# goroda/c3sc

Measured on AMD Instinct MI355X. Metric: Bellman-sweep nodes/sec (7D car rank-10), higher is better.
Workload: dtype f64

## Files before the change

c3sc_amd/csrc/c3sc_hip.hip:

```cpp
#include <hip/hip_runtime.h>

#include <algorithm>
#include <cmath>
#include <cstdio>
#include <cstdlib>
#include <cstring>
#include <string>
#include <vector>

#include "../../include/c3sc_hip.h"
#include "fiber_partition.hpp"
#include "fiber_partition_sort.hpp"
#include "kernel_chain_walk.hpp"
#include "kernel_common.hpp"
#include "kernel_rollout.hpp"
#include "kernel_rollout_ode.hpp"
#include "model_tables.hpp"
#include "pad_cores.hpp"
#include "registry.hpp"

namespace c3sc {

std::vector<KernelEntry> &kernel_registry()
{
// ... 929 lines not shown
    A.h2 = c->h2;
    A.discount = c->discount;
    for (int i = 0; i < 2 * c->d; i++) A.t[i] = c->t[i];
    for (int i = 0; i < C3SC_MAX_PARAMS; i++) A.prm[i] = c->prm[i];
    A.status = c->d_status;
    A.game_gsz = c->game_gsz;
    A.game_ngrp = c->game_ngrp;
    A.game_order = c->game_order;
    A.hz_off = c->hz_dt > 0.0 ? c->hz_off : 0;
    {
        static const int dbg_env = [] { const char *e = getenv("C3SC_DBG"); return e ? atoi(e) : 0; }();
        A.dbg = dbg_env;
        if (dbg_env && !c->d_dbg) { HIPCHK(c, hipMalloc((void **)&c->d_dbg, 65536 * 8 * sizeof(unsigned long long))); }
        A.dbgbuf = c->d_dbg;
        if (A.dbg & 8) A.ncand = 1;
        if (A.dbg & 16) A.ncand = 3;
    }
    return C3SC_OK;
}

static void arm_memo(c3sc_hip_ctx *c, const KernelEntry *e, KArgs &A)
{
    A.memo_keys = nullptr;
    if (c->memo.keys == nullptr || e->variant != C3SC_VARIANT_FIBER_PER_WAVE) return;
    A.memo_keys = c->memo.keys; A.memo_vals = c->memo.vals; A.memo_capmask = c->memo.capmask; A.memo_epoch_bits = c->memo.epoch_bits;
    A.memo_shift = c->memo.shift; A.memo_counters = c->memo.counters; A.memo_mode = c->memo.mode;
    for (int m = 0; m < c->d; m++) A.memo_stride[m] = c->memo.stride[m];
    c->memo.applied = true;
}

static hipError_t ctx_launch(const c3sc_hip_ctx *c, const KernelEntry &e, const KArgs &A, LaunchIO io)
{
    io.form = c->switches;
    return launch_entry(e, A, io);
}

static int launch_one(c3sc_hip_ctx *c, const KernelEntry *e, const KArgs &A, const LaunchIO &io, const char *unsupported = nullptr)
{
    c->last_kernel = e->name;
    g_launches++;
    c->status_cache_valid = false;
    const hipError_t he = ctx_launch(c, *e, A, io);
    if (he == hipErrorNotSupported && unsupported) return fail(c, C3SC_ERR_UNSUPPORTED, unsupported);
    HIPCHK(c, he);
    return C3SC_OK;
}

constexpr long FIBER_PARTITION_MIN = 262144;
static long fiber_partition_min()
{
    const char *e = getenv("C3SC_FIBER_PARTITION");
    if (!e || !*e) return FIBER_PARTITION_MIN;
    const long v = atol(e);
    return v > 0 ? v : -1;
}

static long fiber_group_floor()
{
    const char *e = getenv("C3SC_FIBER_GROUP");
    if (!e || !*e) return FPART_MIN_PER_BIN;
    const long v = atol(e);
    return v > 0 ? v : -1;
}

static bool fiber_rank()
{
// ... 1041 lines not shown
```

c3sc_amd/csrc/inst_car7d_fpp.hip:

```cpp
#include "launch_fpw.hpp"
#include "launch_fpp.hpp"
#include "models.hpp"
namespace c3sc {
#define REG7P(RP)                                  \
    C3SC_REG_FPP1(C3SC_MODEL_CAR7D, RP, 0, Car7D)  \
    C3SC_REG_FPP1(C3SC_MODEL_CAR7D, RP, 1, Car7D)  \
    C3SC_REG_FPP1(C3SC_MODEL_CAR7D, RP, 2, Car7D)  \
    C3SC_REG_FPP1(C3SC_MODEL_CAR7D, RP, 3, Car7D)  \
    C3SC_REG_FPP1(C3SC_MODEL_CAR7D, RP, 4, Car7D)  \
    C3SC_REG_FPP1(C3SC_MODEL_CAR7D, RP, 5, Car7D)  \
    C3SC_REG_FPP1(C3SC_MODEL_CAR7D, RP, 6, Car7D)
#define CAR7_MAP(K, MERGED, NVEC)                                                                   \
    static_assert(PairPark<Car7D, K>::merged() == (MERGED), "car7d: merged dimensions of K = " #K); \
    static_assert(PairMap<Car7D, K>::nv() == (NVEC), "car7d: folded vectors of K = " #K);
CAR7_MAP(0, 0x1Eu, 5)
CAR7_MAP(1, 0x1Du, 6)
CAR7_MAP(2, 0x18u, 9)
CAR7_MAP(3, 0x04u, 11)
CAR7_MAP(4, 0x0Bu, 7)
CAR7_MAP(5, 0x0Fu, 5)
CAR7_MAP(6, 0x17u, 5)
C3SC_FPP_TABLE3(Car7D, 10)
#define CAR7_PLAN3(K, ROUNDS, PRODUCTS)                                                                                  \
    static_assert(PairMap<Car7D, K, true, true>::plan().staged == (ROUNDS), "car7d: three-core staging rounds of K = " #K); \
    static_assert(PairMap<Car7D, K, true, true>::plan().products == (PRODUCTS), "car7d: three-core products of K = " #K);
CAR7_PLAN3(0, 3, 24)
CAR7_PLAN3(1, 2, 16)
CAR7_PLAN3(2, 1, 8)
CAR7_PLAN3(3, 0, 0)
CAR7_PLAN3(4, 1, 6)
CAR7_PLAN3(5, 2, 8)
CAR7_PLAN3(6, 3, 16)
REG7P(4)
REG7P(10)
}
```

c3sc_amd/csrc/kernel_fiber_pair.hpp:

```cpp
#pragma once
#include <utility>

#include "fold_lds.hpp"

#ifndef FPP_CGD
#define FPP_CGD 3
#endif
#ifndef FPP_PIPE2
#define FPP_PIPE2 1
#endif
#ifndef FPP_CG
#define FPP_CG 1
#endif
#ifndef FPP_NV
#define FPP_NV 4
#endif

#ifndef FPP_DIRECT_MAXD
#define FPP_DIRECT_MAXD 3
#endif
#ifndef FPP_EDGE_TABLES
#define FPP_EDGE_TABLES 1
#endif

#ifndef FPP_NODE_SPLIT
#define FPP_NODE_SPLIT 1
#endif
#ifndef FPP_NODE_SPLIT_VGPRS
#define FPP_NODE_SPLIT_VGPRS 140
#endif

namespace c3sc {

constexpr int FPP_THREADS = 128;

template <class Model, int RP>
__host__ __device__ constexpr bool fpp_direct() { return Model::D <= FPP_DIRECT_MAXD && RP <= 8; }

template <class Model, int RP>
__host__ __device__ constexpr bool fpp_edge_tables() { return FPP_EDGE_TABLES && !fpp_direct<Model, RP>() && Model::D >= 4; }

template <int RP>
__device__ __forceinline__ void load_row16(const double *__restrict__ p, double (&r)[RP])
{
    typedef double v2d __attribute__((ext_vector_type(2)));
#pragma unroll
    for (int i = 0; i < RP / 2; i++) {
        const v2d v = *reinterpret_cast<const v2d *>(p + 2 * i);
        r[2 * i] = v.x;
        r[2 * i + 1] = v.y;
    }
}

template <int RP, int NW, int FIRST, int COUNT, bool ROWVEC>
__device__ inline void apply_core_and(const double *G, double (&W)[NW][RP], double (&E)[RP])
{
    constexpr int N1 = COUNT >= FPP_NV - 1 ? FPP_NV - 1 : COUNT;
    double tmp[N1 + 1][RP];
#pragma unroll
    for (int a = 0; a < RP; a++) tmp[0][a] = E[a];
#pragma unroll
    for (int s = 0; s < N1; s++)
// ... 249 lines not shown
    {
        if (PK::merged() == 0u) return pair_owner<K>(it);
        int load[2] = {0, 0}, own[NIT] = {};
        bool done[NIT] = {};
        for (int n = 0; n < NIT; n++) {
            int best = -1;
            for (int q = 0; q < NIT; q++)
                if (valid(q) && !done[q] && (best < 0 || cost(q) > cost(best))) best = q;
            if (best < 0) break;
            const int h = load[1] < load[0] ? 1 : 0;
            own[best] = h;
            load[h] += cost(best);
            done[best] = true;
        }
        return own[it];
    }
    template <int H>
    __host__ __device__ static constexpr int lslot(int it)
    {
        return (it == UL || it < K) ? SL::template slot<H>(it) : SR::template slot<H>(it);
    }
};

__host__ __device__ constexpr bool fpp_node_split_optout(int d, int rp, int k) { return rp < 10 || (d == 7 && rp == 10 && k == 4); }
template <class Model, int RP, int K>
__host__ __device__ constexpr bool fpp_node_split()
{
    if constexpr (!FPP_NODE_SPLIT || fpp_direct<Model, RP>()) return false;
    else
        return PairPark<Model, K>::merged() != 0u && PairMap<Model, K>::nv() * RP * 2 <= FPP_NODE_SPLIT_VGPRS &&
               !fpp_node_split_optout(Model::D, RP, K);
}

template <class Model, int K>
struct PairPre {
    static constexpr unsigned MASK = PairPark<Model, K>::merged(), RATES = PairPark<Model, K>::rates();
    const double *PX;
    int lane;
    double pvc;
    __device__ inline double q() const { return PX[PairPark<Model, K>::row_q() * 64 + lane]; }
    __device__ inline double pv() const { return pvc; }
    __device__ inline double pm(int m) const { return PX[PairPark<Model, K>::row_pm(m) * 64 + lane]; }
    __device__ inline double pp(int m) const { return PX[(PairPark<Model, K>::row_pm(m) + 1) * 64 + lane]; }
};

#define FPP_STAMP(slot)                                                   \
    if (C3SC_STAMPS_ON && (A.dbg & 128)) {                                \
        const unsigned long long now__ = clock64();                       \
        seg[slot] += now__ - tlast;                                       \
        tlast = now__;                                                    \
    }

template <class Model, int RP, int K, int H, bool PART, bool T3, bool LEFT, int m, int NOWN, class Combine>
__device__ __attribute__((always_inline)) inline void fold_step(const KArgs &A, const double *__restrict__ ro, double *sK,
                                                               const int (&fi)[Model::D], const int (&nbm)[Model::D], const int (&nbp)[Model::D],
                                                               const double (&rpm)[Model::D], const double (&rpp)[Model::D], double (&V)[RP],
                                                               double (&W)[NOWN][RP], unsigned long long (&seg)[12], unsigned long long &tlast,
                                                               Combine &&combine)
{
    constexpr int D = Model::D;
    constexpr bool DIRECT = fpp_direct<Model, RP>();
    typedef PairMap<Model, K, fpp_edge_tables<Model, RP>(), T3> PM;
    typedef typename PM::template Side<LEFT> SD;
    constexpr bool RV = SD::ROWVEC;
    constexpr int BASE = SD::template base<H>();
    constexpr KeyLevels KL = fpp_group_levels(D, RP, K);
// ... 29 lines not shown
                vecmat_lds<RP, 1>(src + nbm[m] * str, t0);
                vecmat_lds<RP, 1>(src + nbp[m] * str, t1);
            } else {
                matvec_lds<RP, 1>(src + nbm[m] * str, t0);
                matvec_lds<RP, 1>(src + nbp[m] * str, t1);
            }
#pragma unroll
            for (int a = 0; a < RP; a++) {
                if constexpr (PAIR) { W[BASE + before][a] = t0[0][a]; W[BASE + before + 1][a] = t1[0][a]; }
                else nw[a] = fma(rpp[m], t1[0][a], rpm[m] * t0[0][a]);
            }
        }
        if constexpr (DIRECT) {
            double tl[1][RP];
#pragma unroll
            for (int a = 0; a < RP; a++) tl[0][a] = V[a];
            apply_glb<RP, 1, RV>(G, tl);
#pragma unroll
            for (int a = 0; a < RP; a++) V[a] = tl[0][a];
            apply_range_glb<RP, NOWN, BASE, before, RV>(G, W);
        } else if constexpr (UNI)
            apply_uni_and<RP, NOWN, BASE, before, RV>(G, W, V);
        else
            apply_core_and<RP, NOWN, BASE, before, RV>(G, W, V);
        if constexpr (ACC) {
            constexpr int su = SD::template slot<H>(SD::U);
#pragma unroll
            for (int a = 0; a < RP; a++) W[su][a] = (m == SD::first_merged()) ? nw[a] : W[su][a] + nw[a];
        }
    };
    fold_level<GROUP && (m == KL.major || (KL.n > 1 && m == KL.minor))>(fi[m], body);
}

template <class Model, int RP, int K, int H, bool FORCED, bool PART, bool T3 = false>
__device__ __attribute__((always_inline)) inline void fiber_pair_body(const KArgs &A, const double *__restrict__ ro,
                                                                     const int32_t *__restrict__ idx, double *__restrict__ outv,
                                                                     int32_t *__restrict__ uidx, int32_t *__restrict__ absorbed,
                                                                     const int32_t *__restrict__ perm, const int32_t *__restrict__ nlive_p,
                                                                     double *sK, unsigned &st)
{
    constexpr int D = Model::D;
    constexpr int S = 2 * D + 1;
    constexpr int RH = RP / 2;
    typedef PairPark<Model, K> PK;
    constexpr bool ET = fpp_edge_tables<Model, RP>();
    typedef PairMap<Model, K, ET, T3> PM;
    static_assert(!T3 || (PART && ET), "the three-core tables serve the partitioned kernels with edge tables");
    static_assert(PM::nv() == PairMap<Model, K, ET>::nv() && PM::gslot(D + 1) == PairMap<Model, K, ET>::gslot(D + 1),
                  "the table depth moves no slot of the node loop");
    constexpr FoldPlan PL = PM::plan();
    constexpr int NV = PM::nv();
    constexpr int NVL = PM::SL::nv();
    constexpr int NOL = PM::SL::template before<H>(K);
    constexpr int NOR = PM::SR::template before<H>(K);
    constexpr int NOWN = (NOL + NOR) > 0 ? (NOL + NOR) : 1;
    constexpr int NP = NV + 1;
    constexpr bool DIRECT = fpp_direct<Model, RP>();
    constexpr KeyLevels KL = fpp_group_levels(D, RP, K);
    constexpr bool GROUP = PART && KL.n > 0;
    static_assert(!GROUP || fpp_key_levels(D, K, ET).major == KL.major, "the key levels follow the kernel's own fold plan");
    static_assert(RP % 2 == 0, "rank-split kernel needs an even padded rank");
    const int lane = threadIdx.x & 63;
    const int N = A.N;
    const long ntiles = (A.F + 63) / 64;
    int first_dead = 0x7fffffff;
    if constexpr (PART) first_dead = __builtin_amdgcn_readfirstlane((int)(((long)*nlive_p + 63) >> 6));
    unsigned long long seg[12] = {0, 0, 0, 0, 0, 0, 0, 0, 0, 0, 0, 0}, tlast = clock64();
    CandLds<Model> cr;
    NodeLds<Model, K> nr;
    {
        CandRegs<Model> cr0;
        cr0.load(A, ro);
        NodeRegs<Model, K> nr0;
        nr0.load(A, ro);
        double *tb = sK + A.tbl_off;
        cr.fill(tb, cr0, A.ncand);
        nr.fill(tb + CandLds<Model>::doubles(A.ncand), nr0, N);
        pair_barrier();
    }

    for (long tile = blockIdx.x; tile < ntiles; tile += gridDim.x) {
        FPP_STAMP(7)
        const long f_raw = tile * 64 + lane;
        const bool live = f_raw < A.F;
        const long f_pos = live ? f_raw : A.F - 1;
        long f = f_pos;
        if constexpr (PART) f = (long)perm[f_pos];
        const bool dead_tile = PART && tile >= (long)first_dead;

        if constexpr (PART) if (dead_tile) {
            const bool whole = A.bctype[K] == C3SC_ABSORB || A.cends != 0;
            const int jb = whole ? 0 : 1, je = whole ? N : N - 1;
            double xb[D];
#pragma unroll
            for (int m = 0; m < D; m++) xb[m] = (m != K && PK::need_x(m)) ? ro[A.xg_off[m] + idx[f * D + m]] : 0.0;
            for (int j = jb + ((jb ^ H) & 1); j < je; j += 2) {
                xb[K] = nr.x_at(j);
                outv[(size_t)f * N + j] = Model::boundcost(A.prm, xb);
                if (uidx) uidx[(size_t)f * N + j] = -1;
                if (absorbed) absorbed[(size_t)f * N + j] = 1;
            }
            if (whole) continue;
        }

        int fi[D], nbm[D], nbp[D];
        bool fiber_abs = false;
        double x[D];
#pragma unroll
        for (int m = 0; m < D; m++) {
            fi[m] = (m == K) ? 0 : idx[f * D + m];
            const bool face = fixed_neighbors(fi[m], A.ngrid[m], A.bctype[m], nbm[m], nbp[m]);
            if (m != K) fiber_abs = fiber_abs || face;
            x[m] = ro[A.xg_off[m] + fi[m]];
        }

        const unsigned obs_fixed = obstacle_mask_fixed<D>(A, ro, x, K);
        double tv[Model::NTAB > 0 ? Model::NTAB : 1];
        table_values<Model>(A, ro, fi, tv);

        double rpm[D], rpp[D];
#pragma unroll
        for (int m = 0; m < D; m++) { rpm[m] = 0.0; rpp[m] = 0.0; }
        if constexpr (PK::constd() != 0) {
            typename Model::Node nd0;
            Model::prep(A.prm, x, tv, nd0);
            double u0[Model::DU], cf0[Model::NCF > 0 ? Model::NCF : 1], b0[D], s0[D];
#pragma unroll
            for (int i = 0; i < Model::DU; i++) u0[i] = cr.get_u(i, 0);
            cf0[0] = 0.0;
#pragma unroll
            for (int i = 0; i < Model::NCF; i++) cf0[i] = cr.get_cf(i, 0);
            Model::drift(A.prm, nd0, x, u0, cf0, b0);
            Model::sigma(A.prm, x, u0, s0);
#pragma unroll
            for (int m = 0; m < D; m++)
                if ((PK::constd() >> m) & 1u) upwind_rates(A.t[2 * m], A.t[2 * m + 1], b0[m], s0[m], rpm[m], rpp[m]);
        }

        double L[RP], R[RP], W[NOWN][RP];
#pragma unroll
        for (int a = 0; a < RP; a++) { L[a] = (a == 0) ? 1.0 : 0.0; R[a] = (a == 0) ? 1.0 : 0.0; }

        auto side3 = [&](auto lc, double (&V)[RP]) __attribute__((always_inline)) {
            constexpr bool LEFT = decltype(lc)::value;
            typedef typename PM::template Side<LEFT> SD;
            constexpr int c0 = SD::core(0), c1 = SD::core(1), c2 = SD::core(2);
            constexpr int BASE = SD::template base<H>();
            const double *T = ro + (LEFT ? pair_tab3L_off(A, RP) : pair_tab3R_off(A, RP));
            const int n0 = A.ngrid[c0], n1 = A.ngrid[c1];
            auto row = [&](int j0, int j1, int j2) __attribute__((always_inline)) -> const double * {
                return T + (LEFT ? ((long)j2 * n0 + j0) * n1 + j1 : ((long)j2 * n1 + j1) * n0 + j0) * RP;
            };
            constexpr bool OWN0 = SD::template owns<H>(c0), OWN1 = SD::template owns<H>(c1), OWN2 = SD::template owns<H>(c2);
            double tm[3][RP], tp[3][RP];
            load_row16<RP>(row(fi[c0], fi[c1], fi[c2]), V);
            if constexpr (OWN0) {
                load_row16<RP>(row(nbm[c0], fi[c1], fi[c2]), tm[0]);
                load_row16<RP>(row(nbp[c0], fi[c1], fi[c2]), tp[0]);
            }
            if constexpr (OWN1) {
                load_row16<RP>(row(fi[c0], nbm[c1], fi[c2]), tm[1]);
                load_row16<RP>(row(fi[c0], nbp[c1], fi[c2]), tp[1]);
            }
            if constexpr (OWN2) {
                load_row16<RP>(row(fi[c0], fi[c1], nbm[c2]), tm[2]);
                load_row16<RP>(row(fi[c0], fi[c1], nbp[c2]), tp[2]);
            }
            __builtin_amdgcn_sched_barrier(0);
            auto combine = [&]() __attribute__((always_inline)) {
// ... 131 lines not shown
            if constexpr (PM::SR::tab() && K == PL.rfirst) right_combine();
            if constexpr (!PM::SR::tab()) {
                constexpr bool GLB = DIRECT || !PL.redge;
                constexpr int str = GLB ? RP : fpl_lds_stride(RP);
                const double *src = sK;
                FPP_STAMP(1)
                if constexpr (GLB) src = ro + A.core_off[D - 1];
                else {
                    pair_barrier();
                    stage_core_image<H>(sK, A.img_base + A.pair_img_off[D - 1], A.ngrid[D - 1] * str);
                    pair_barrier();
                }
                FPP_STAMP(7)
#pragma unroll
                for (int a = 0; a < RP; a++) {
                    R[a] = src[fi[D - 1] * str + a];
                    if constexpr (PM::mg(D - 1)) {
                        if constexpr (PM::owner(PM::UR) == H)
                            W[NOL][a] = fma(rpp[D - 1], src[nbp[D - 1] * str + a], rpm[D - 1] * src[nbm[D - 1] * str + a]);
                    } else if constexpr (PM::owner(D - 1) == H) {
                        W[NOL][a] = src[nbm[D - 1] * str + a];
                        W[NOL + 1][a] = src[nbp[D - 1] * str + a];
                    }
                }
            }
            auto right_step = [&](auto mc) __attribute__((always_inline)) {
                fold_step<Model, RP, K, H, PART, T3, false, decltype(mc)::value>(A, ro, sK, fi, nbm, nbp, rpm, rpp, R, W, seg, tlast, right_combine);
            };
            static_for<PM::SR::nsteps()>([&](auto ic) __attribute__((always_inline)) { right_step(std::integral_constant<int, PM::SR::step(decltype(ic)::value)>{}); });
        }

        }
        FPP_STAMP(1)
        constexpr bool NS = fpp_node_split<Model, RP, K>();
        double Wh[NS ? 1 : NV][RH];
        double Wf[NS ? NV : 1][RP];
        if constexpr (NS) {
            double *X = sK;
            auto put_get_own = [&](auto ic, auto pc) __attribute__((always_inline)) {
                constexpr int it = decltype(ic)::value, P = decltype(pc)::value;
                if constexpr (PM::valid(it) && PM::owner(it) == H) {
                    constexpr int slot = PM::template lslot<H>(it);
#pragma unroll
                    for (int s = 0; s < PM::count(it); s++) {
                        const int g = PM::gslot(it) + s;
#pragma unroll
                        for (int i = 0; i < RH; i++) {
                            X[(g * RH + i) * 64 + lane] = W[slot + s][P * RH + i];
                            Wf[g][P * RH + i] = W[slot + s][P * RH + i];
                        }
                    }
                }
            };
            auto get_other = [&](auto ic, auto pc) __attribute__((always_inline)) {
                constexpr int it = decltype(ic)::value, P = decltype(pc)::value;
                if constexpr (PM::valid(it) && PM::owner(it) != H) {
#pragma unroll
                    for (int s = 0; s < PM::count(it); s++) {
                        const int g = PM::gslot(it) + s;
#pragma unroll
                        for (int i = 0; i < RH; i++) Wf[g][P * RH + i] = X[(g * RH + i) * 64 + lane];
                    }
                }
            };
            auto half = [&](auto pc) __attribute__((always_inline)) {
                pair_barrier();
                static_for<PM::NIT>([&](auto ic) __attribute__((always_inline)) { put_get_own(ic, pc); });
                pair_barrier();
                static_for<PM::NIT>([&](auto ic) __attribute__((always_inline)) { get_other(ic, pc); });
            };
// ... 5 lines not shown
            pair_barrier();
            auto put_get_own = [&](auto ic) __attribute__((always_inline)) {
                constexpr int it = decltype(ic)::value;
                if constexpr (PM::valid(it) && PM::owner(it) == H) {
                    constexpr int slot = PM::template lslot<H>(it);
#pragma unroll
                    for (int s = 0; s < PM::count(it); s++) {
                        const int g = PM::gslot(it) + s;
#pragma unroll
                        for (int i = 0; i < RH; i++) {
                            X[(g * RH + i) * 64 + lane] = W[slot + s][(1 - H) * RH + i];
                            Wh[g][i] = W[slot + s][H * RH + i];
                        }
                    }
                }
            };
            static_for<PM::NIT>(put_get_own);
            pair_barrier();
            auto get_other = [&](auto ic) __attribute__((always_inline)) {
                constexpr int it = decltype(ic)::value;
                if constexpr (PM::valid(it) && PM::owner(it) != H) {
#pragma unroll
                    for (int s = 0; s < PM::count(it); s++) {
                        const int g = PM::gslot(it) + s;
#pragma unroll
                        for (int i = 0; i < RH; i++) Wh[g][i] = X[(g * RH + i) * 64 + lane];
                    }
                }
            };
            static_for<PM::NIT>(get_other);
            pair_barrier();
        }
        double *sL = sK, *sR = sK + RP * 64;
        {
#pragma unroll
            for (int a = 0; a < RP; a++) {
                if constexpr (H == 0) sL[a * 64 + lane] = L[a];
                else sR[a * 64 + lane] = R[a];
            }
            if constexpr (H == 0) {
                static_assert(PK::rows() <= NP, "parking rows exceed the reserved block");
                double *PXw = sK + (2 * RP + 2 * (NP + 1) + NP) * 64;
#pragma unroll
                for (int m = 0; m < D; m++)
                    if (PK::need_x(m)) PXw[PK::row_x(m) * 64 + lane] = x[m];
#pragma unroll
                for (int t = 0; t < Model::NTAB; t++)
                    if (PK::need_t(t)) PXw[PK::row_t(t) * 64 + lane] = tv[t];
#pragma unroll
                for (int m = 0; m < D; m++)
                    if ((PK::rates() >> m) & 1u) {
                        PXw[PK::row_pm(m) * 64 + lane] = rpm[m];
                        PXw[(PK::row_pm(m) + 1) * 64 + lane] = rpp[m];
                    }
                if constexpr (PK::merged() != 0u) {
                    double qc = 0.0;
#pragma unroll
                    for (int m = 0; m < D; m++)
                        if (PM::mg(m)) { qc += rpm[m]; qc += rpp[m]; }
                    PXw[PK::row_q() * 64 + lane] = qc;
                }
            }
            pair_barrier();
        }
        FPP_STAMP(2)

        const int bck = A.bctype[K];
        const double *Gk = ro + A.core_off[K];
        auto partials = [&](int j, auto &&sink) __attribute__((always_inline)) -> double {
            double pv;
            if constexpr (K == 0) {
                double ah[RH];
#pragma unroll
                for (int i = 0; i < RH; i++) ah[i] = Gk[(size_t)j * RP + H * RH + i];
                double v = 0.0;
#pragma unroll
                for (int i = 0; i < RH; i++) v = fma(ah[i], sR[(H * RH + i) * 64 + lane], v);
                pv = v;
#pragma unroll
                for (int g = 0; g < NV; g++) sink(g, dot_reg<RH>(ah, Wh[g]));
            } else if constexpr (K == D - 1) {
                double ch[RH];
#pragma unroll
                for (int i = 0; i < RH; i++) ch[i] = Gk[(size_t)j * RP + H * RH + i];
                double v = 0.0;
#pragma unroll
                for (int i = 0; i < RH; i++) v = fma(sL[(H * RH + i) * 64 + lane], ch[i], v);
                pv = v;
// ... 80 lines not shown
                for (int i = 0; i < RH; i++)
#pragma unroll
                    for (int a = 0; a < BH; a++) asm volatile("" : "+s"(g[i][a]));
#pragma unroll
                for (int a = 0; a < BH; a++) {
                    if (a0 + a < RP) {
                        const double la = vec[a0 + a];
#pragma unroll
                        for (int i = 0; i < RH; i++) ah[i] = fma(la, g[i][a], ah[i]);
                    }
                }
            }
        };
        auto dots_quarter = [&](int q, const double (&ch)[RH], const double (&ah)[RH], auto &&sink) __attribute__((always_inline)) {
#pragma unroll
            for (int g = 0; g < NV; g++)
                if (g * 4 / NV == q) sink(g, (g < NVL) ? dot_reg<RH>(Wh[g], ch) : dot_reg<RH>(ah, Wh[g]));
        };
        auto dots_part = [&](const double (&ch)[RH], const double (&ah)[RH], auto &&sink) __attribute__((always_inline)) -> double {
            double v = 0.0;
#pragma unroll
            for (int i = 0; i < RH; i++) v = fma(sL[(H * RH + i) * 64 + lane], ch[i], v);
#pragma unroll
            for (int g = 0; g < NVL; g++) sink(g, dot_reg<RH>(Wh[g], ch));
#pragma unroll
            for (int g = NVL; g < NV; g++) sink(g, dot_reg<RH>(ah, Wh[g]));
            sink(NV, v);
            return v;
        };
        double *B0 = sK + 2 * RP * 64;
        double *B1 = B0 + (NP + 1) * 64;
        double *B2 = B1 + (NP + 1) * 64;
        double *PX = B2 + NP * 64;

        auto finalize = [&](int jn, const double (&Vt)[NP], double vlo, double vhi) __attribute__((always_inline)) {
            double V[S];
#pragma unroll
            for (int m = 0; m < D; m++) {
                if (m == K) { V[2 * m] = vlo; V[2 * m + 1] = vhi; }
                else if (PM::mg(m)) { V[2 * m] = 0.0; V[2 * m + 1] = 0.0; }
                else { V[2 * m] = Vt[PM::gslot(m)]; V[2 * m + 1] = Vt[PM::gslot(m) + 1]; }
            }
            V[2 * D] = Vt[NV];
            double pvc = 0.0;
            if constexpr (PM::valid(PM::UL)) pvc += Vt[PM::gslot(PM::UL)];
            if constexpr (PM::valid(PM::UR)) pvc += Vt[PM::gslot(PM::UR)];
            double x[D], tv[Model::NTAB > 0 ? Model::NTAB : 1];
            tv[0] = 0.0;
#pragma unroll
            for (int m = 0; m < D; m++)
                x[m] = (m == K) ? nr.x_at(jn) : (PairPark<Model, K>::need_x(m) ? PX[PairPark<Model, K>::row_x(m) * 64 + lane] : 0.0);
#pragma unroll
            for (int t = 0; t < Model::NTAB; t++)
                tv[t] = (Model::tab_dim(t) == K) ? nr.tab_at(t, jn)
                                                 : (PairPark<Model, K>::need_t(t) ? PX[PairPark<Model, K>::row_t(t) * 64 + lane] : 0.0);
            int ab = (obs_fixed & nr.mask_at(jn)) ? -1 : 0;
            if (fiber_abs) ab = 1;
            int lo, hi;
            ab = vary_neighbors(jn, N, bck, ab, lo, hi, A.cends);
            int ui;
            FPP_STAMP(8)
            int fu = -1;
            if constexpr (FORCED) fu = A.forced[(size_t)f * N + jn];
            const PairPre<Model, K> pre{PX, lane, pvc};
            const double val = node_backup<Model, FPP_CG, FPP_CGD, CandLds<Model>, true, PairPre<Model, K>>(A, ro, x, tv, cr, V, ab, ui, st, FORCED, fu, pre);
            FPP_STAMP(9)
// ... 26 lines not shown
                constexpr int NE = RP * RP, NB = (NE + 3) / 4;
                double c[RP], a[RP], lv[RP];
#pragma unroll
                for (int i = 0; i < RP; i++) lv[i] = sL[i * 64 + lane];
#pragma unroll
                for (int i = 0; i < RP; i++) { c[i] = 0.0; a[i] = 0.0; }
#pragma unroll
                for (int b0 = 0; b0 < NE; b0 += NB) {
                    double g[NB];
#pragma unroll
                    for (int e = 0; e < NB; e++) g[e] = (b0 + e < NE) ? G0[b0 + e] : 0.0;
                    double rv[RP];
#pragma unroll
                    for (int p = 0; p < RP; p++) rv[p] = (p >= b0 / RP && p * RP < b0 + NB) ? sR[p * 64 + lane] : 0.0;
                    __builtin_amdgcn_sched_barrier(0);
#pragma unroll
                    for (int e = 0; e < NB; e++) asm volatile("" : "+s"(g[e]));
#pragma unroll
                    for (int e = 0; e < NB; e++) {
                        if (b0 + e < NE) {
                            const int p = (b0 + e) / RP, q = (b0 + e) % RP;
                            c[q] = fma(g[e], rv[p], c[q]);
                            a[p] = fma(lv[q], g[e], a[p]);
                        }
                    }
#pragma unroll
                    for (int i = 0; i < RP; i++) asm volatile("" : "+v"(c[i]), "+v"(a[i]));
                }
#pragma unroll
                for (int i = 0; i < RP; i++) v = fma(sL[i * 64 + lane], c[i], v);
#pragma unroll
                for (int g = 0; g < NVL; g++) Vt[g] = dot_reg<RP>(Wf[g], c);
#pragma unroll
                for (int g = NVL; g < NV; g++) Vt[g] = dot_reg<RP>(a, Wf[g]);
            }
            Vt[NV] = v;
        };
        double *VX = B0;
        double vwrap = 0.0;
        if (bck == C3SC_PERIODIC) {
            double Vw[NP];
            stencil(N - 2, Vw);
            vwrap = Vw[NV];
        }
        double vone = 0.0;
        double v_m2 = 0.0, v_m1 = 0.0;
        double Vd[NP];
#pragma unroll
        for (int g = 0; g < NP; g++) Vd[g] = 0.0;
        const int T = N / 2 + 1;
        for (int t = 0; t < T; t++) {
            const int j0 = 2 * t, j1 = 2 * t + 1;
            const bool has0 = j0 < N, has1 = j1 < N;
            double *vx = VX + (t & 1) * 64;
            double v0 = 0.0, v1 = 0.0;
            double Pn[NP];
#pragma unroll
            for (int g = 0; g < NP; g++) Pn[g] = 0.0;
            if constexpr (H == 0) {
                if (has0) {
                    stencil(j0, Pn);
                    v0 = Pn[NV];
                    vx[lane] = v0;
                }
                FPP_STAMP(3)
                pair_barrier();
                FPP_STAMP(4)
// ... 166 lines not shown
    if (h == 0) fiber_pair_body<Model, RP, K, 0, FORCED, false>(A, ro, idx, outv, uidx, absorbed, nullptr, nullptr, sKp, st);
    else fiber_pair_body<Model, RP, K, 1, FORCED, false>(A, ro, idx, outv, uidx, absorbed, nullptr, nullptr, sKp, st);
    if (st) atomicOr(A.status, st);
}

template <class Model, int RP, int K, bool FORCED>
__global__ void __launch_bounds__(FPP_THREADS, (fpp_waves_per_simd<Model, RP>()))
    k_fiber_pair_part(const KArgs A, const double *__restrict__ ro, const int32_t *__restrict__ idx, double *__restrict__ outv,
                      int32_t *__restrict__ uidx, int32_t *__restrict__ absorbed, const int32_t *__restrict__ perm,
                      const int32_t *__restrict__ nlive_p)
{
    extern __shared__ double sKp[];
    unsigned st = 0;
    const int h = __builtin_amdgcn_readfirstlane(threadIdx.x >> 6);
    if (h == 0) fiber_pair_body<Model, RP, K, 0, FORCED, true>(A, ro, idx, outv, uidx, absorbed, perm, nlive_p, sKp, st);
    else fiber_pair_body<Model, RP, K, 1, FORCED, true>(A, ro, idx, outv, uidx, absorbed, perm, nlive_p, sKp, st);
    if (st) atomicOr(A.status, st);
}

template <class Model, int RP, int K, bool FORCED>
__global__ void __launch_bounds__(FPP_THREADS, (fpp_waves_per_simd<Model, RP>()))
    k_fiber_pair_part3(const KArgs A, const double *__restrict__ ro, const int32_t *__restrict__ idx, double *__restrict__ outv,
                       int32_t *__restrict__ uidx, int32_t *__restrict__ absorbed, const int32_t *__restrict__ perm,
                       const int32_t *__restrict__ nlive_p)
{
    extern __shared__ double sKp[];
    unsigned st = 0;
    const int h = __builtin_amdgcn_readfirstlane(threadIdx.x >> 6);
    if (h == 0) fiber_pair_body<Model, RP, K, 0, FORCED, true, true>(A, ro, idx, outv, uidx, absorbed, perm, nlive_p, sKp, st);
    else fiber_pair_body<Model, RP, K, 1, FORCED, true, true>(A, ro, idx, outv, uidx, absorbed, perm, nlive_p, sKp, st);
    if (st) atomicOr(A.status, st);
}

}
```

c3sc_amd/csrc/launch_fpp.hpp:

```cpp
#pragma once
#include "kernel_fiber_pair.hpp"
#include "registry.hpp"

namespace c3sc {

template <class Model, int RP, int K>
__host__ __device__ constexpr size_t fpp_tile_doubles(bool node_split)
{
    constexpr int NV = PairMap<Model, K>::nv(), NP = NV + 1, RH = RP / 2;
    const size_t swap = (size_t)NV * RH * 64;
    const size_t parked = (size_t)(2 * RP + (NP + 1) * 2 + NP) * 64;
    const size_t rows = node_split ? parked + (size_t)PairPark<Model, K>::rows() * 64 : parked + (size_t)NP * 64;
    return swap > rows ? swap : rows;
}

template <class Model, int RP>
struct FppTable3 {
    static constexpr bool value = false;
};
#define C3SC_FPP_TABLE3(MODEL, RP)                                                                                              \
    template <>                                                                                                                 \
    struct FppTable3<MODEL, RP> {                                                                                               \
        static constexpr bool value = true;                                                                                     \
        static_assert(fpp_table3_registered(MODEL::D, RP) && fpp_edge_tables<MODEL, RP>(), "the host reserves no tables here"); \
    };
template <class Model, int RP, int K>
constexpr bool fpp_table3() { return FppTable3<Model, RP>::value && !fpp_table3_optout(Model::D, RP, K); }

template <class Model, int RP, int K, bool FORCED, bool PART, bool T3 = false>
hipError_t launch_fpp_impl(const KArgs &A, const LaunchIO &io)
{
    constexpr int D = Model::D;
    if (A.ncand > 64) return hipErrorNotSupported;
    constexpr bool NS = fpp_node_split<Model, RP, K>();
    static_assert(fpp_tile_doubles<Model, RP, K>(NS) <= fpp_tile_doubles<Model, RP, K>(false), "the node split must not need more LDS than the rank split");
    static_assert(!NS || 4 * fpp_tile_doubles<Model, RP, K>(NS) * sizeof(double) <= 160 * 1024, "four node-split workgroups per CU must fit the LDS");
    size_t doubles = fpp_tile_doubles<Model, RP, K>(false);
    for (int m = 0; m < D; m++) {
        if (m == K || fpp_direct<Model, RP>()) continue;
        const int elems = (m == 0 || m == D - 1) ? RP : RP * RP;
        const size_t need = ((size_t)A.ngrid[m] * fpl_lds_stride(elems) + 1) & ~(size_t)1;
        if (need > doubles) doubles = need;
    }
    KArgs B = A;
    B.tbl_off = (int)doubles;
    doubles += (size_t)CandLds<Model>::doubles(A.ncand) + (size_t)NodeLds<Model, K>::doubles(A.N);
    const size_t shmem = doubles * sizeof(double);
    static_assert(!T3 || PART, "the three-core kernel is a partitioned one");
    const void *kern = PART ? (const void *)k_fiber_pair_part<Model, RP, K, FORCED> : (const void *)k_fiber_pair<Model, RP, K, FORCED>;
    if constexpr (T3) kern = (const void *)k_fiber_pair_part3<Model, RP, K, FORCED>;
    static LaunchCache cache;
    int blocks_per_cu = 1, num_cu = 256;
    hipError_t e = cache.prepare(kern, FPP_THREADS, shmem, blocks_per_cu, num_cu);
    if (e != hipSuccess) return e;
    const long ntiles = (A.F + 63) / 64;
    const long cap = (long)num_cu * blocks_per_cu;
    int grid = (int)(ntiles < cap ? ntiles : cap);
    if (ntiles >= 8 * cap && ntiles < 0x7fffffffL) grid = (int)ntiles;
    if (grid < 1) grid = 1;
    if constexpr (T3)
        hipLaunchKernelGGL((k_fiber_pair_part3<Model, RP, K, FORCED>), dim3(grid), dim3(FPP_THREADS), shmem, io.stream, B, io.ro, io.idx, io.out,
                           io.uidx, io.absorbed, io.perm, io.nlive);
    else if constexpr (PART)
        hipLaunchKernelGGL((k_fiber_pair_part<Model, RP, K, FORCED>), dim3(grid), dim3(FPP_THREADS), shmem, io.stream, B, io.ro, io.idx, io.out,
                           io.uidx, io.absorbed, io.perm, io.nlive);
    else
        hipLaunchKernelGGL((k_fiber_pair<Model, RP, K, FORCED>), dim3(grid), dim3(FPP_THREADS), shmem, io.stream, B, io.ro, io.idx, io.out, io.uidx,
                           io.absorbed);
    return hipGetLastError();
}

template <class Model, int RP, int K>
hipError_t launch_fpp(const KArgs &A, const LaunchIO &io)
{
    if constexpr (fpp_table3<Model, RP, K>())
        if (io.perm && io.tab3) return A.forced ? launch_fpp_impl<Model, RP, K, true, true, true>(A, io) : launch_fpp_impl<Model, RP, K, false, true, true>(A, io);
    if (io.perm) return A.forced ? launch_fpp_impl<Model, RP, K, true, true>(A, io) : launch_fpp_impl<Model, RP, K, false, true>(A, io);
    return A.forced ? launch_fpp_impl<Model, RP, K, true, false>(A, io) : launch_fpp_impl<Model, RP, K, false, false>(A, io);
}

#define C3SC_REG_FPP1(MODEL_ID, RP, K, ...)                                                                   \
    static Registrar C3SC_CAT(reg_fpp_, __COUNTER__)(KernelEntry{                                             \
        MODEL_ID, __VA_ARGS__::D, RP, 0, C3SC_VARIANT_FIBER_PAIR, 128, K, &launch_fpp<__VA_ARGS__, RP, K>, \
        "k_fiber_pair<" #__VA_ARGS__ "," #RP ",K=" #K ">"});

}
```

c3sc_amd/csrc/registry.hpp:

```cpp
#pragma once
#ifndef __HIPCC_RTC__
#include <hip/hip_runtime.h>

#include <mutex>
#include <vector>
#endif

#include "kernel_common.hpp"

namespace c3sc {

#ifndef __HIPCC_RTC__
struct LaunchIO {
    const double *ro;
    const int32_t *idx;
    double *out;
    int32_t *uidx;
    int32_t *absorbed;
    const int32_t *nbf;
    const int32_t *nbv;
    const double *tbl;
    const double *tcost;
    hipStream_t stream;
    const void *sim = nullptr;
    const int32_t *perm = nullptr;
    const int32_t *nlive = nullptr;
    bool tab3 = false;
    unsigned form = 0;
};
#endif

constexpr int VARIANT_ROLLOUT = 100, VARIANT_STENCIL_POINTS = 101, VARIANT_ROLLOUT_ODE = 102;
constexpr int VARIANT_CHAIN_WALK = 103, VARIANT_CHAIN_TRANSITIONS = 104;
__host__ __device__ constexpr bool is_fiber_variant(int v) { return v < VARIANT_ROLLOUT; }

#ifndef __HIPCC_RTC__
struct RtcLaunch;

typedef hipError_t (*launch_fn)(const KArgs &A, const LaunchIO &io);

struct KernelEntry {
    int model;
    int d;
    int rp;
    int npl;
    int variant;
    int max_n;
    int k;
    launch_fn fn;
    const char *name;
    const RtcLaunch *rtc = nullptr;
};

std::vector<KernelEntry> &kernel_registry();

struct LaunchCache {
    static constexpr int MAXDEV = 16;
    std::mutex mu;
    size_t attr_shmem[MAXDEV] = {0}, occ_shmem[MAXDEV] = {0};
    int blocks_per_cu[MAXDEV] = {0}, num_cu[MAXDEV] = {0};
// ... 49 lines not shown
```

Measured before the change: 35.04 billion.

## Park excess folded vectors in LDS for car7d rank-10 K=2,4 pair kernels

```diff
diff --git a/c3sc_amd/csrc/c3sc_hip.hip b/c3sc_amd/csrc/c3sc_hip.hip
--- a/c3sc_amd/csrc/c3sc_hip.hip
+++ b/c3sc_amd/csrc/c3sc_hip.hip
@@ -985,6 +985,8 @@
 static hipError_t ctx_launch(const c3sc_hip_ctx *c, const KernelEntry &e, const KArgs &A, LaunchIO io)
 {
     io.form = c->switches;
+    const char *pk = getenv("C3SC_PAIR_PARKED");
+    io.parked = !(pk && *pk && atol(pk) == 0);
     return launch_entry(e, A, io);
 }
 
diff --git a/c3sc_amd/csrc/inst_car7d_fpp.hip b/c3sc_amd/csrc/inst_car7d_fpp.hip
--- a/c3sc_amd/csrc/inst_car7d_fpp.hip
+++ b/c3sc_amd/csrc/inst_car7d_fpp.hip
@@ -31,6 +31,8 @@
 CAR7_PLAN3(4, 1, 6)
 CAR7_PLAN3(5, 2, 8)
 CAR7_PLAN3(6, 3, 16)
+C3SC_FPP_PARKED(Car7D, 10, 2)
+C3SC_FPP_PARKED(Car7D, 10, 4)
 REG7P(4)
 REG7P(10)
 }
diff --git a/c3sc_amd/csrc/inst_car7d_fpp_pk.hip b/c3sc_amd/csrc/inst_car7d_fpp_pk.hip
--- /dev/null
+++ b/c3sc_amd/csrc/inst_car7d_fpp_pk.hip
@@ -0,0 +1,16 @@
+#include "launch_fpp.hpp"
+#include "models.hpp"
+namespace c3sc {
+#define CAR7_PARKED(K, P, HOME, ROWS)                                                                                       \
+    static_assert(fpp_parked<Car7D, 10, K>() == (P), "car7d: parked vectors of K = " #K);                                  \
+    static_assert(fpp_parked_home_row<Car7D, 10, K>() == (HOME) && fpp_parked_rows<Car7D, 10, K>() == (ROWS), "car7d: rows of K = " #K); \
+           \
+    static_assert(fpp_tile_doubles<Car7D, 10, K>(true, true) <= fpp_tile_doubles<Car7D, 10, K>(false), "car7d: LDS of K = " #K); \
+    static_assert(fpp_tile_doubles<Car7D, 10, K>(true, true) <= (size_t)41 * fpl_lds_stride(10 * 10), "car7d: staged image, K = " #K);
+CAR7_PARKED(2, 3, 31, 61)
+CAR7_PARKED(4, FPP_PARKED_K4, 31, 31 + 10 * FPP_PARKED_K4)
+static_assert(fpp_parked<Car7D, 10, 0>() == 0 && fpp_parked<Car7D, 10, 1>() == 0 && fpp_parked<Car7D, 10, 3>() == 0 &&
+              fpp_parked<Car7D, 10, 5>() == 0 && fpp_parked<Car7D, 10, 6>() == 0, "car7d: every other K keeps its form");
+C3SC_FPP_PARKED_KERNELS(Car7D, 10, 2)
+C3SC_FPP_PARKED_KERNELS(Car7D, 10, 4)
+}
diff --git a/c3sc_amd/csrc/kernel_fiber_pair.hpp b/c3sc_amd/csrc/kernel_fiber_pair.hpp
--- a/c3sc_amd/csrc/kernel_fiber_pair.hpp
+++ b/c3sc_amd/csrc/kernel_fiber_pair.hpp
@@ -28,6 +28,9 @@
 #endif
 #ifndef FPP_NODE_SPLIT_VGPRS
 #define FPP_NODE_SPLIT_VGPRS 140
+#endif
+#ifndef FPP_PARKED_K4
+#define FPP_PARKED_K4 1
 #endif
 
 namespace c3sc {
@@ -343,6 +346,28 @@
                !fpp_node_split_optout(Model::D, RP, K);
 }
 
+__host__ __device__ constexpr int fpp_parked_count(int d, int rp, int k) { return (d == 7 && rp == 10) ? (k == 2 ? 3 : (k == 4 ? FPP_PARKED_K4 : 0)) : 0; }
+template <class Model, int RP, int K>
+__host__ __device__ constexpr int fpp_parked()
+{
+    if constexpr (!FPP_NODE_SPLIT || fpp_direct<Model, RP>() || fpp_node_split<Model, RP, K>()) return 0;
+    else {
+        constexpr int P = PairPark<Model, K>::merged() != 0u ? fpp_parked_count(Model::D, RP, K) : 0;
+        return (P > 0 && PairMap<Model, K>::nv() - P >= PairMap<Model, K>::SL::nv() && PairMap<Model, K>::nv() - P > 0) ? P : 0;
+    }
+}
+template <int RP>
+__host__ __device__ constexpr int fpp_parked_px_row() { return 2 * RP + 4; }
+template <class Model, int RP, int K>
+__host__ __device__ constexpr int fpp_parked_home_row()
+{
+    constexpr int hand = (PairMap<Model, K>::nv() - fpp_parked<Model, RP, K>()) * (RP / 2);
+    constexpr int low = fpp_parked_px_row<RP>() + PairPark<Model, K>::rows();
+    return hand > low ? hand : low;
+}
+template <class Model, int RP, int K>
+__host__ __device__ constexpr int fpp_parked_rows() { return fpp_parked_home_row<Model, RP, K>() + fpp_parked<Model, RP, K>() * RP; }
+
 template <class Model, int K>
 struct PairPre {
     static constexpr unsigned MASK = PairPark<Model, K>::merged(), RATES = PairPark<Model, K>::rates();
@@ -438,7 +463,7 @@
     fold_level<GROUP && (m == KL.major || (KL.n > 1 && m == KL.minor))>(fi[m], body);
 }
 
-template <class Model, int RP, int K, int H, bool FORCED, bool PART, bool T3 = false>
+template <class Model, int RP, int K, int H, bool FORCED, bool PART, bool T3 = false, int PKD = 0>
 __device__ __attribute__((always_inline)) inline void fiber_pair_body(const KArgs &A, const double *__restrict__ ro,
                                                                      const int32_t *__restrict__ idx, double *__restrict__ outv,
                                                                      int32_t *__restrict__ uidx, int32_t *__restrict__ absorbed,
@@ -496,7 +521,12 @@
 
         if constexpr (PART) if (dead_tile) {
             const bool whole = A.bctype[K] == C3SC_ABSORB || A.cends != 0;
-            const int jb = whole ? 0 : 1, je = whole ? N : N - 1;
+            int jb = whole ? 0 : 1;
+            const int je = whole ? N : N - 1;
+            if constexpr (PKD > 0) {
+                asm volatile("" : "+v"(jb));
+                jb = __builtin_amdgcn_readfirstlane(jb);
+            }
             double xb[D];
 #pragma unroll
             for (int m = 0; m < D; m++) xb[m] = (m != K && PK::need_x(m)) ? ro[A.xg_off[m] + idx[f * D + m]] : 0.0;
@@ -540,7 +570,21 @@
             Model::sigma(A.prm, x, u0, s0);
 #pragma unroll
             for (int m = 0; m < D; m++)
-                if ((PK::constd() >> m) & 1u) upwind_rates(A.t[2 * m], A.t[2 * m + 1], b0[m], s0[m], rpm[m], rpp[m]);
+                if ((PK::constd() >> m) & 1u) {
+                    if constexpr (PKD > 0) {
+                        double t2 = A.t[2 * m + 1];
+                        asm volatile("" : "+s"(t2));
+                        upwind_rates(A.t[2 * m], t2, b0[m], s0[m], rpm[m], rpp[m]);
+                    } else
+                        upwind_rates(A.t[2 * m], A.t[2 * m + 1], b0[m], s0[m], rpm[m], rpp[m]);
+                }
+        }
+
+        double qc_pk = 0.0;
+        if constexpr (PKD > 0 && PK::merged() != 0u) {
+#pragma unroll
+            for (int m = 0; m < D; m++)
+                if (PM::mg(m)) { qc_pk += rpm[m]; qc_pk += rpp[m]; }
         }
 
         double L[RP], R[RP], W[NOWN][RP];
@@ -738,10 +782,63 @@
 
         }
         FPP_STAMP(1)
-        constexpr bool NS = fpp_node_split<Model, RP, K>();
+        constexpr bool NS = fpp_node_split<Model, RP, K>() || PKD > 0;
+        constexpr int NR = NV - PKD;
+        static_assert(PKD == 0 || (PKD == fpp_parked<Model, RP, K>() && K > 0 && K < D - 1 && NR >= NVL && !T3), "parked slots are right of a middle K");
         double Wh[NS ? 1 : NV][RH];
-        double Wf[NS ? NV : 1][RP];
-        if constexpr (NS) {
+        double Wf[NS ? NR : 1][RP];
+        double *HM = sK;
+        if constexpr (PKD > 0) {
+            typedef double v2d __attribute__((ext_vector_type(2)));
+            double *X = sK;
+            HM = sK + fpp_parked_home_row<Model, RP, K>() * 64;
+            static_assert(fpp_parked_home_row<Model, RP, K>() >= NR * RH, "homes above the hand-over rows");
+            auto put_get_own = [&](auto ic, auto pc) __attribute__((always_inline)) {
+                constexpr int it = decltype(ic)::value, P = decltype(pc)::value;
+                if constexpr (PM::valid(it) && PM::owner(it) == H) {
+                    constexpr int slot = PM::template lslot<H>(it);
+                    static_for<PM::count(it)>([&](auto sc) __attribute__((always_inline)) {
+                        constexpr int s = decltype(sc)::value, g = PM::gslot(it) + s;
+                        if constexpr (g < NR) {
+#pragma unroll
+                            for (int i = 0; i < RH; i++) {
+                                X[(g * RH + i) * 64 + lane] = W[slot + s][P * RH + i];
+                                Wf[g][P * RH + i] = W[slot + s][P * RH + i];
+                            }
+                        } else if constexpr (P == 0) {
+#pragma unroll
+                            for (int i = 0; i < RH; i++) {
+                                v2d t;
+                                t.x = W[slot + s][2 * i];
+                                t.y = W[slot + s][2 * i + 1];
+                                *reinterpret_cast<v2d *>(HM + (((g - NR) * RH + i) * 64 + lane) * 2) = t;
+                            }
+                        }
+                    });
+                }
+            };
+            auto get_other = [&](auto ic, auto pc) __attribute__((always_inline)) {
+                constexpr int it = decltype(ic)::value, P = decltype(pc)::value;
+                if constexpr (PM::valid(it) && PM::owner(it) != H) {
+                    static_for<PM::count(it)>([&](auto sc) __attribute__((always_inline)) {
+                        constexpr int g = PM::gslot(it) + decltype(sc)::value;
+                        if constexpr (g < NR) {
+#pragma unroll
+                            for (int i = 0; i < RH; i++) Wf[g][P * RH + i] = X[(g * RH + i) * 64 + lane];
+                        }
+                    });
+                }
+            };
+            auto half = [&](auto pc) __attribute__((always_inline)) {
+                pair_barrier();
+                static_for<PM::NIT>([&](auto ic) __attribute__((always_inline)) { put_get_own(ic, pc); });
+                pair_barrier();
+                static_for<PM::NIT>([&](auto ic) __attribute__((always_inline)) { get_other(ic, pc); });
+            };
+            half(std::integral_constant<int, 0>{});
+            half(std::integral_constant<int, 1>{});
+            pair_barrier();
+        } else if constexpr (NS) {
             double *X = sK;
             auto put_get_own = [&](auto ic, auto pc) __attribute__((always_inline)) {
                 constexpr int it = decltype(ic)::value, P = decltype(pc)::value;
@@ -813,6 +910,14 @@
             pair_barrier();
         }
         double *sL = sK, *sR = sK + RP * 64;
+        if constexpr (PKD > 0) {
+            int ln = lane;
+            asm volatile("" : "+v"(ln));
+            const long fr2 = tile * 64 + ln;
+            const long fp2 = fr2 < A.F ? fr2 : A.F - 1;
+            f = fp2;
+            if constexpr (PART) f = (long)perm[fp2];
+        }
         {
 #pragma unroll
             for (int a = 0; a < RP; a++) {
@@ -821,20 +926,37 @@
             }
             if constexpr (H == 0) {
                 static_assert(PK::rows() <= NP, "parking rows exceed the reserved block");
-                double *PXw = sK + (2 * RP + 2 * (NP + 1) + NP) * 64;
+                double *PXw = sK + (PKD > 0 ? fpp_parked_px_row<RP>() : 2 * RP + 2 * (NP + 1) + NP) * 64;
+                if constexpr (PKD > 0) {
+                    long fr = f;
+                    asm volatile("" : "+v"(fr));
+                    int fi2[D];
+#pragma unroll
+                    for (int m = 0; m < D; m++) fi2[m] = (m == K || !(PK::need_x(m) || PK::nt() > 0)) ? 0 : idx[fr * D + m];
+                    double tv2[Model::NTAB > 0 ? Model::NTAB : 1];
+                    table_values<Model>(A, ro, fi2, tv2);
+#pragma unroll
+                    for (int m = 0; m < D; m++)
+                        if (PK::need_x(m)) PXw[PK::row_x(m) * 64 + lane] = ro[A.xg_off[m] + fi2[m]];
+#pragma unroll
+                    for (int t = 0; t < Model::NTAB; t++)
+                        if (PK::need_t(t)) PXw[PK::row_t(t) * 64 + lane] = tv2[t];
+                } else {
 #pragma unroll
                 for (int m = 0; m < D; m++)
                     if (PK::need_x(m)) PXw[PK::row_x(m) * 64 + lane] = x[m];
 #pragma unroll
                 for (int t = 0; t < Model::NTAB; t++)
                     if (PK::need_t(t)) PXw[PK::row_t(t) * 64 + lane] = tv[t];
+                }
 #pragma unroll
                 for (int m = 0; m < D; m++)
                     if ((PK::rates() >> m) & 1u) {
                         PXw[PK::row_pm(m) * 64 + lane] = rpm[m];
                         PXw[(PK::row_pm(m) + 1) * 64 + lane] = rpp[m];
                     }
-                if constexpr (PK::merged() != 0u) {
+                if constexpr (PKD > 0 && PK::merged() != 0u) PXw[PK::row_q() * 64 + lane] = qc_pk;
+                else if constexpr (PK::merged() != 0u) {
                     double qc = 0.0;
 #pragma unroll
                     for (int m = 0; m < D; m++)
@@ -981,6 +1103,8 @@
         double *B1 = B0 + (NP + 1) * 64;
         double *B2 = B1 + (NP + 1) * 64;
         double *PX = B2 + NP * 64;
+        if constexpr (PKD > 0) PX = sK + fpp_parked_px_row<RP>() * 64;
+        static_assert(PKD == 0 || fpp_parked_px_row<RP>() + PK::rows() <= fpp_parked_home_row<Model, RP, K>(), "the parked rows end below the homes");
 
         auto finalize = [&](int jn, const double (&Vt)[NP], double vlo, double vhi) __attribute__((always_inline)) {
             double V[S];
@@ -1073,7 +1197,21 @@
 #pragma unroll
                 for (int g = 0; g < NVL; g++) Vt[g] = dot_reg<RP>(Wf[g], c);
 #pragma unroll
-                for (int g = NVL; g < NV; g++) Vt[g] = dot_reg<RP>(a, Wf[g]);
+                for (int g = NVL; g < NR; g++) Vt[g] = dot_reg<RP>(a, Wf[g]);
+                if constexpr (PKD > 0) {
+                    typedef double v2d __attribute__((ext_vector_type(2)));
+#pragma unroll
+                    for (int p = 0; p < PKD; p++) {
+                        double w[RP];
+#pragma unroll
+                        for (int i = 0; i < RH; i++) {
+                            const v2d t = *reinterpret_cast<const v2d *>(HM + ((p * RH + i) * 64 + lane) * 2);
+                            w[2 * i] = t.x;
+                            w[2 * i + 1] = t.y;
+                        }
+                        Vt[NR + p] = dot_reg<RP>(a, w);
+                    }
+                }
             }
             Vt[NV] = v;
         };
@@ -1306,4 +1444,35 @@
     if (st) atomicOr(A.status, st);
 }
 
-}
+template <class Model, int RP, int K, bool FORCED>
+__global__ void __launch_bounds__(FPP_THREADS, (fpp_waves_per_simd<Model, RP>()))
+    k_fiber_pair_pk(const KArgs A, const double *__restrict__ ro, const int32_t *__restrict__ idx, double *__restrict__ outv,
+                    int32_t *__restrict__ uidx, int32_t *__restrict__ absorbed)
+{
+    extern __shared__ double sKp[];
+    constexpr int P = fpp_parked<Model, RP, K>();
+    static_assert(P > 0, "no parked node split for this instantiation");
+    unsigned st = 0;
+    const int h = __builtin_amdgcn_readfirstlane(threadIdx.x >> 6);
+    if (h == 0) fiber_pair_body<Model, RP, K, 0, FORCED, false, false, P>(A, ro, idx, outv, uidx, absorbed, nullptr, nullptr, sKp, st);
+    else fiber_pair_body<Model, RP, K, 1, FORCED, false, false, P>(A, ro, idx, outv, uidx, absorbed, nullptr, nullptr, sKp, st);
+    if (st) atomicOr(A.status, st);
+}
+
+template <class Model, int RP, int K, bool FORCED>
+__global__ void __launch_bounds__(FPP_THREADS, (fpp_waves_per_simd<Model, RP>()))
+    k_fiber_pair_part_pk(const KArgs A, const double *__restrict__ ro, const int32_t *__restrict__ idx, double *__restrict__ outv,
+                         int32_t *__restrict__ uidx, int32_t *__restrict__ absorbed, const int32_t *__restrict__ perm,
+                         const int32_t *__restrict__ nlive_p)
+{
+    extern __shared__ double sKp[];
+    constexpr int P = fpp_parked<Model, RP, K>();
+    static_assert(P > 0, "no parked node split for this instantiation");
+    unsigned st = 0;
+    const int h = __builtin_amdgcn_readfirstlane(threadIdx.x >> 6);
+    if (h == 0) fiber_pair_body<Model, RP, K, 0, FORCED, true, false, P>(A, ro, idx, outv, uidx, absorbed, perm, nlive_p, sKp, st);
+    else fiber_pair_body<Model, RP, K, 1, FORCED, true, false, P>(A, ro, idx, outv, uidx, absorbed, perm, nlive_p, sKp, st);
+    if (st) atomicOr(A.status, st);
+}
+
+}
diff --git a/c3sc_amd/csrc/launch_fpp.hpp b/c3sc_amd/csrc/launch_fpp.hpp
--- a/c3sc_amd/csrc/launch_fpp.hpp
+++ b/c3sc_amd/csrc/launch_fpp.hpp
@@ -1,12 +1,16 @@
 #pragma once
+#include <cstdio>
+#include <cstdlib>
+
 #include "kernel_fiber_pair.hpp"
 #include "registry.hpp"
 
 namespace c3sc {
 
 template <class Model, int RP, int K>
-__host__ __device__ constexpr size_t fpp_tile_doubles(bool node_split)
+__host__ __device__ constexpr size_t fpp_tile_doubles(bool node_split, bool pk = false)
 {
+    if (pk) return (size_t)fpp_parked_rows<Model, RP, K>() * 64;
     constexpr int NV = PairMap<Model, K>::nv(), NP = NV + 1, RH = RP / 2;
     const size_t swap = (size_t)NV * RH * 64;
     const size_t parked = (size_t)(2 * RP + (NP + 1) * 2 + NP) * 64;
@@ -27,7 +31,14 @@
 template <class Model, int RP, int K>
 constexpr bool fpp_table3() { return FppTable3<Model, RP>::value && !fpp_table3_optout(Model::D, RP, K); }
 
-template <class Model, int RP, int K, bool FORCED, bool PART, bool T3 = false>
+template <class Model, int RP, int K>
+struct FppParked {
+    static constexpr bool value = false;
+};
+template <class Model, int RP, int K>
+constexpr bool fpp_parked_registered() { return FppParked<Model, RP, K>::value && fpp_parked<Model, RP, K>() > 0; }
+
+template <class Model, int RP, int K, bool FORCED, bool PART, bool T3 = false, bool PK = false>
 hipError_t launch_fpp_impl(const KArgs &A, const LaunchIO &io)
 {
     constexpr int D = Model::D;
@@ -36,6 +47,12 @@
     static_assert(fpp_tile_doubles<Model, RP, K>(NS) <= fpp_tile_doubles<Model, RP, K>(false), "the node split must not need more LDS than the rank split");
     static_assert(!NS || 4 * fpp_tile_doubles<Model, RP, K>(NS) * sizeof(double) <= 160 * 1024, "four node-split workgroups per CU must fit the LDS");
     size_t doubles = fpp_tile_doubles<Model, RP, K>(false);
+    if constexpr (PK) {
+        static_assert(!T3 && fpp_parked<Model, RP, K>() > 0, "a parked kernel where the form is used, behind the two-core tables");
+        constexpr size_t pk = fpp_tile_doubles<Model, RP, K>(true, true);
+        static_assert(4 * (pk * sizeof(double) + 1560) <= 160 * 1024, "four parked workgroups per CU must fit the LDS");
+        if (pk > doubles) doubles = pk;
+    }
     for (int m = 0; m < D; m++) {
         if (m == K || fpp_direct<Model, RP>()) continue;
         const int elems = (m == 0 || m == D - 1) ? RP : RP * RP;
@@ -47,18 +64,28 @@
     doubles += (size_t)CandLds<Model>::doubles(A.ncand) + (size_t)NodeLds<Model, K>::doubles(A.N);
     const size_t shmem = doubles * sizeof(double);
     static_assert(!T3 || PART, "the three-core kernel is a partitioned one");
-    const void *kern = PART ? (const void *)k_fiber_pair_part<Model, RP, K, FORCED> : (const void *)k_fiber_pair<Model, RP, K, FORCED>;
-    if constexpr (T3) kern = (const void *)k_fiber_pair_part3<Model, RP, K, FORCED>;
+    const void *kern = nullptr;
+    if constexpr (PK)
+        kern = PART ? (const void *)k_fiber_pair_part_pk<Model, RP, K, FORCED> : (const void *)k_fiber_pair_pk<Model, RP, K, FORCED>;
+    else if constexpr (T3) kern = (const void *)k_fiber_pair_part3<Model, RP, K, FORCED>;
+    else kern = PART ? (const void *)k_fiber_pair_part<Model, RP, K, FORCED> : (const void *)k_fiber_pair<Model, RP, K, FORCED>;
     static LaunchCache cache;
     int blocks_per_cu = 1, num_cu = 256;
     hipError_t e = cache.prepare(kern, FPP_THREADS, shmem, blocks_per_cu, num_cu);
     if (e != hipSuccess) return e;
+    if (PK && getenv("C3SC_VERBOSE")) fprintf(stderr, "c3sc: parked node split K=%d: %zu B of LDS, %d workgroups per CU\n", K, shmem, blocks_per_cu);
     const long ntiles = (A.F + 63) / 64;
     const long cap = (long)num_cu * blocks_per_cu;
     int grid = (int)(ntiles < cap ? ntiles : cap);
     if (ntiles >= 8 * cap && ntiles < 0x7fffffffL) grid = (int)ntiles;
     if (grid < 1) grid = 1;
-    if constexpr (T3)
+    if constexpr (PK && PART)
+        hipLaunchKernelGGL((k_fiber_pair_part_pk<Model, RP, K, FORCED>), dim3(grid), dim3(FPP_THREADS), shmem, io.stream, B, io.ro, io.idx, io.out,
+                           io.uidx, io.absorbed, io.perm, io.nlive);
+    else if constexpr (PK)
+        hipLaunchKernelGGL((k_fiber_pair_pk<Model, RP, K, FORCED>), dim3(grid), dim3(FPP_THREADS), shmem, io.stream, B, io.ro, io.idx, io.out, io.uidx,
+                           io.absorbed);
+    else if constexpr (T3)
         hipLaunchKernelGGL((k_fiber_pair_part3<Model, RP, K, FORCED>), dim3(grid), dim3(FPP_THREADS), shmem, io.stream, B, io.ro, io.idx, io.out,
                            io.uidx, io.absorbed, io.perm, io.nlive);
     else if constexpr (PART)
@@ -71,8 +98,26 @@
 }
 
 template <class Model, int RP, int K>
+hipError_t launch_fpp_parked(const KArgs &A, const LaunchIO &io)
+{
+    if (io.perm) return A.forced ? launch_fpp_impl<Model, RP, K, true, true, false, true>(A, io) : launch_fpp_impl<Model, RP, K, false, true, false, true>(A, io);
+    return A.forced ? launch_fpp_impl<Model, RP, K, true, false, false, true>(A, io) : launch_fpp_impl<Model, RP, K, false, false, false, true>(A, io);
+}
+#define C3SC_FPP_PARKED(MODEL, RP, K)                                                                        \
+    template <>                                                                                              \
+    struct FppParked<MODEL, RP, K> {                                                                         \
+        static constexpr bool value = true;                                                                  \
+        static_assert(fpp_parked<MODEL, RP, K>() > 0, "no parked node split for this instantiation");        \
+    };                                                                                                       \
+    extern template hipError_t launch_fpp_parked<MODEL, RP, K>(const KArgs &, const LaunchIO &);
+#define C3SC_FPP_PARKED_KERNELS(MODEL, RP, K) template hipError_t launch_fpp_parked<MODEL, RP, K>(const KArgs &, const LaunchIO &);
+
+template <class Model, int RP, int K>
 hipError_t launch_fpp(const KArgs &A, const LaunchIO &io)
 {
+    static_assert(!(fpp_parked_registered<Model, RP, K>() && fpp_table3<Model, RP, K>()), "one replacement kernel per K");
+    if constexpr (fpp_parked_registered<Model, RP, K>())
+        if (io.parked) return launch_fpp_parked<Model, RP, K>(A, io);
     if constexpr (fpp_table3<Model, RP, K>())
         if (io.perm && io.tab3) return A.forced ? launch_fpp_impl<Model, RP, K, true, true, true>(A, io) : launch_fpp_impl<Model, RP, K, false, true, true>(A, io);
     if (io.perm) return A.forced ? launch_fpp_impl<Model, RP, K, true, true>(A, io) : launch_fpp_impl<Model, RP, K, false, true>(A, io);
diff --git a/c3sc_amd/csrc/registry.hpp b/c3sc_amd/csrc/registry.hpp
--- a/c3sc_amd/csrc/registry.hpp
+++ b/c3sc_amd/csrc/registry.hpp
@@ -26,6 +26,7 @@
     const int32_t *perm = nullptr;
     const int32_t *nlive = nullptr;
     bool tab3 = false;
+    bool parked = true;
     unsigned form = 0;
 };
 #endif
```

Result: faster. 36.13 billion, median of 6 (+3.1%).
